# zrlhahaha/Direct12PBRRenderer

Hardware: AMD Instinct MI355X
Metric: shaded Mpixel/s at 4K G-buffer (full deferred frame: clustered shade + bloom + auto-exposure + ACES) (higher is better)
Workload: dtype f32

## Files before the change

### direct12pbrrenderer_amd/csrc/bloom.hip

```cpp
#include <type_traits>
#include "pbr_internal.hpp"
#include "pbr_device.hpp"

using namespace pbr;

__constant__ float c_gauss[9] = {0.0148f, 0.0459f, 0.1050f, 0.1941f, 0.2803f, 0.1941f, 0.1050f, 0.0459f, 0.0148f};

__device__ __forceinline__ float4 to4(F4 v) { return make_float4(v.x, v.y, v.z, v.w); }
__device__ __forceinline__ F4 from4(float4 v) { return f4(v.x, v.y, v.z, v.w); }

struct OutRect { int x0, y0, x1, y1, ox, oy, pitch; };
constexpr int PF_MAX_RECTS = 5;
struct OutRects {
    int n, ox, oy, pitch;
    int x0[PF_MAX_RECTS], y0[PF_MAX_RECTS], x1[PF_MAX_RECTS], y1[PF_MAX_RECTS], tiles_x[PF_MAX_RECTS], first[PF_MAX_RECTS + 1];
};
__global__ __launch_bounds__(256) void k_bloom_prefilter(const pbr_half* __restrict__ hdr, int w, int h, int pitch,
                                                           pbr_half* __restrict__ out, OutRect rc,
                                                           float tx, float ty, float threshold, float knee) {
    const int x = rc.x0 + blockIdx.x * 64 + threadIdx.x;
    const int y = rc.y0 + blockIdx.y * 4 + threadIdx.y;
    if (x >= rc.x1 || y >= rc.y1) return;
    const float u = (float)x * tx, v = (float)y * ty;
    const float ox[5] = {0.0f, -1.0f, -1.0f, 1.0f, 1.0f};
// ... 378 lines not shown
        float fx, hfx, hfy = 0.0f;
        float4 smp[PER_T];
        int ax0, ax1, bx0, bx1;
        tap1d<MODE>(x0 - 4 + lane, iw, ax0, ax1, fx);
        tap1d<MODE>(x0 - 4 + hc, iw, bx0, bx1, hfx);
        const int sx = clampi(x0 - 4 + lane, 0, ow - 1), shx = clampi(x0 - 4 + hc, 0, ow - 1);
        const int first = y0 - 4 + r0;
        const bool shared_rows = MODE == M_UP && first >= 1 && first + PER_T - 1 <= oh - 2;
        if (MODE == M_UP && shared_rows) {
            constexpr int NR = PER_T / 2 + 2;
            const int base = (first >> 1) - 1 + (first & 1);
            V3 hrow[NR];
            const float wx0 = 1.0f - fx;
#pragma unroll
            for (int j = 0; j < NR; j++) {
                const H4* row = reinterpret_cast<const H4*>(in) + (size_t)min(base + j, ih - 1) * iw;
                const H4 c0 = row[ax0], c1 = row[ax1];
                hrow[j] = fma3(h3f(c1), fx, h3f(c0) * wx0);
            }
            auto blend = [&](auto parity) {
                constexpr int P = decltype(parity)::value;
#pragma unroll
                for (int k = 0; k < PER_T; k++) {
                    constexpr int dummy = 0; (void)dummy;
                    const int odd = (P + k) & 1;
                    const int i0 = (P + k + 1) / 2 - P;
                    const float fyk = odd ? 0.25f : 0.75f, wy0 = 1.0f - fyk;
                    const V3 r = fma3(hrow[i0 + 1], fyk, hrow[i0] * wy0);
                    smp[k] = make_float4(r.x, r.y, r.z, 0.0f);
                }
            };
            if (first & 1) blend(std::integral_constant<int, 1>{}); else blend(std::integral_constant<int, 0>{});
#pragma unroll
            for (int k = 0; k < PER_T; k++)
                if (DUAL) up[k] = reinterpret_cast<const H4*>(in2)[(size_t)(first + k) * ow + sx];
        } else {
            Tap2 taps[PER_T];
            float fy[PER_T];
#pragma unroll
            for (int k = 0; k < PER_T; k++) {
                const int jj = clampi(first + k, 0, oh - 1);
                int ay0, ay1;
                tap1d<MODE>(jj, ih, ay0, ay1, fy[k]);
                taps[k] = load_tap2<MODE>(in, iw, ax0, ax1, ay0, ay1);
                if (DUAL) up[k] = reinterpret_cast<const H4*>(in2)[(size_t)jj * ow + sx];
            }
#pragma unroll
            for (int k = 0; k < PER_T; k++) smp[k] = finish_tap2_rgb<MODE>(taps[k], fx, fy[k]);
        }
        if (has_halo) {
            const int jj = clampi(first + hk, 0, oh - 1);
            int ay0, ay1;
            tap1d<MODE>(jj, ih, ay0, ay1, hfy);
            htap = load_tap2<MODE>(in, iw, bx0, bx1, ay0, ay1);
            if (DUAL) hup = reinterpret_cast<const H4*>(in2)[(size_t)jj * ow + shx];
        }
#pragma unroll
        for (int k = 0; k < PER_T; k++) {
            line[lane] = smp[k];
            if (DUAL) line2[lane] = make_float4((float)up[k].x, (float)up[k].y, (float)up[k].z, 0.0f);
            if (has_halo && hk == k) {
                line[hc] = finish_tap2_rgb<MODE>(htap, hfx, hfy);
                if (DUAL) line2[hc] = make_float4((float)hup.x, (float)hup.y, (float)hup.z, 0.0f);
            }
            wave_sync();
            V3 g = gauss9_rgb(line + lane);
            if (DUAL) g = g + gauss9_rgb(line2 + lane);
            wave_sync();
            H4 th;
            th.x = to_half_rn(g.x); th.y = to_half_rn(g.y); th.z = to_half_rn(g.z); th.w = alpha_t;
            sT[r0 + k][lane] = th;
        }
    }
    __syncthreads();
#pragma unroll
    for (int k = 0; k < PER_O; k++) {
        const int r = wv + NW * k, y = y0 + r;
        if (x >= ow || y >= oh) continue;
        V3 a3 = v3(0.0f, 0.0f, 0.0f);
#pragma unroll
        for (int i = 0; i < 9; i++) a3 = fma3(h3f(sT[r + i][lane]), c_gauss[i], a3);
        const F4 a = f4(a3.x, a3.y, a3.z, alpha_v);
        if (TAIL == 0) {
            store_h4(out + 4 * ((size_t)y * out_pitch + x), a);
        } else {
            if (!(in_mx && y >= tr.my0 && y < tr.my1)) continue;
            const half4v a0 = round_h4(a);
            const F4 s = h4f(hdr_in[k]);
            H4 o;
            o.x = to_half_rn(s.x + (float)a0.x); o.y = to_half_rn(s.y + (float)a0.y); o.z = to_half_rn(s.z + (float)a0.z); o.w = to_half_rn(s.w + (float)a0.w);
            *reinterpret_cast<H4*>(out + 4 * ((size_t)(y - tr.by) * out_pitch + (x - tr.bx))) = o;
            if (TAIL == 2) {
                if (x >= tr.hx0 && x < tr.hx1 && y >= tr.hy0 && y < tr.hy1)
                    atomicAdd(&sh_hist[wv][luminance_bin_exact((float)o.x, (float)o.y, (float)o.z, min_log, inv_range)], 1u);
            }
        }
    }
    if (tile + (int)gridDim.x < n_tiles) __syncthreads();
    }
    if (TAIL == 2) {
        __syncthreads();
        for (int i = t; i < PBR_HISTOGRAM_BINS; i += NT) {
            uint32_t sum = 0;
#pragma unroll
            for (int w2 = 0; w2 < NW; w2++) sum += sh_hist[w2][i];
            if (sum) atomicAdd(&hist[i], sum);
        }
    }
}

__device__ __forceinline__ H4 ld_h4(const void* base, uint32_t byte_off) {
    return *reinterpret_cast<const H4*>(reinterpret_cast<const char*>(base) + byte_off);
}
__device__ __forceinline__ void gauss9_pair(const float2* e, float& ge, float& go) {
    const float s[10] = {e[0].x, e[0].y, e[1].x, e[1].y, e[2].x, e[2].y, e[3].x, e[3].y, e[4].x, e[4].y};
    float a = 0.0f, b = 0.0f;
#pragma unroll
    for (int i = 0; i < 9; i++) { a = __builtin_fmaf(s[i], c_gauss[i], a); b = __builtin_fmaf(s[i + 1], c_gauss[i], b); }
    ge = a; go = b;
}

namespace poly {
constexpr double G[9] = {0.0148, 0.0459, 0.1050, 0.1941, 0.2803, 0.1941, 0.1050, 0.0459, 0.0148};
constexpr double g(int k) { return (k < -4 || k > 4) ? 0.0 : G[k + 4]; }
constexpr float E(int j) { return (float)(0.75 * g(2 * j) + 0.25 * g(2 * j + 2) + 0.75 * g(2 * j + 1) + 0.25 * g(2 * j - 1)); }
}

template <bool DUAL, int TAIL, int TH>
__global__ __launch_bounds__(512, 4) void k_blur_up_poly(const pbr_half* __restrict__ in, int iw, int ih,
                                                          const pbr_half* __restrict__ in2,
                                                          pbr_half* __restrict__ out, int ow, int oh, int out_pitch,
                                                          int tiles_x, int n_tiles,
                                                          TailRect tr, float min_log, float inv_range,
                                                          uint32_t* __restrict__ hist) {
    constexpr int TW = 128, NP = TW / 2 + 4, NC = TW / 2 + 6, SR = TH + 8, NT = 512, NW = NT / 64;
    constexpr int NPAIR = TH / 2 + 5;
    constexpr int PPW = (NPAIR + NW - 1) / NW;
    constexpr int PER_O = TH / 4;
    static_assert(TH % 4 == 0 && (PPW + 1) * 6 <= 64 && 2 * PPW * 4 <= 64, "one halo entry per lane");
    __shared__ H4 sLineC[NW][NC + 2];
    __shared__ float2 sLineU[DUAL ? NW : 1][3][NP];
    __shared__ H4 sT[SR][TW];
    __shared__ uint32_t sh_hist[TAIL == 2 ? NW : 1][TAIL == 2 ? PBR_HISTOGRAM_BINS : 1];
    static_assert(sizeof(sLineC) + sizeof(sLineU) + sizeof(sT) + sizeof(sh_hist) <= 80 * 1024, "k_blur_up_poly: two blocks per CU no longer fit the LDS");
    const int t = threadIdx.x, lane = t & 63;
    const int wv = __builtin_amdgcn_readfirstlane(t >> 6);
    const int vc = t & 127, vg = __builtin_amdgcn_readfirstlane(t >> 7);
    if (TAIL == 2) {
        for (int i = t; i < NW * PBR_HISTOGRAM_BINS; i += NT) (&sh_hist[0][0])[i] = 0u;
    }
    const size_t a_at = (size_t)min(tr.my0 >> 1, ih - 1) * iw + min(tr.mx0 >> 1, iw - 1);
    float alpha_h = gauss9_const((float)reinterpret_cast<const H4*>(in)[a_at].w);
    if (DUAL) alpha_h = alpha_h + gauss9_const((float)reinterpret_cast<const H4*>(in2)[(size_t)min(tr.my0, oh - 1) * ow + min(tr.mx0, ow - 1)].w);
    const h16 alpha_t = to_half_rn(alpha_h);
    const float alpha_v = gauss9_const((float)alpha_t);
    const float a0w = (float)to_half_rn(alpha_v);
    auto wave_sync = [] {
        __builtin_amdgcn_fence(__ATOMIC_RELEASE, "wavefront");
        __builtin_amdgcn_wave_barrier();
        __builtin_amdgcn_fence(__ATOMIC_ACQUIRE, "wavefront");
    };
    for (int tile = blockIdx.x; tile < n_tiles; tile += gridDim.x) {
    const int x0 = (tr.tx0 + tile % tiles_x) * TW, y0 = (tr.ty0 + tile / tiles_x) * TH;
    const int xv = x0 + vc, rbase = vg * PER_O;
    H4 hdr_in[PER_O];
    const bool in_mx = TAIL != 0 && xv >= tr.mx0 && xv < tr.mx1;
    char* const hdr_row0 = reinterpret_cast<char*>(out) + (ptrdiff_t)(y0 + rbase - tr.by) * out_pitch * 8;
    const uint32_t hdr_x = (uint32_t)(xv - tr.bx) * 8u;
    const size_t hdr_pitch = (size_t)out_pitch * 8u;
    {
        const int i_first = wv * PPW;
        const int n_pairs = min(PPW, NPAIR - i_first);
        const int cb = (y0 >> 1) - 3 + i_first;
        const uint32_t ccol = (uint32_t)clampi((x0 >> 1) - 3 + lane, 0, iw - 1) * 8u;
        H4 cr[PPW + 1], chalo{};
        const int hk = lane / 6, hq = 64 + lane % 6;
        const bool has_halo = lane < 6 * (PPW + 1);
        H4 upE[DUAL ? 2 * PPW : 1], upO[DUAL ? 2 * PPW : 1], hupE{}, hupO{};
        const int uk = lane >> 2, uq = 64 + (lane & 3);
        const bool has_uhalo = DUAL && lane < 8 * PPW;
        if (n_pairs > 0) {
#pragma unroll
            for (int k = 0; k <= PPW; k++) {
                const char* row = reinterpret_cast<const char*>(in) + (size_t)clampi(cb + k, 0, ih - 1) * iw * 8u;
                cr[k] = ld_h4(row, ccol);
            }
            if (has_halo) {
                const char* row = reinterpret_cast<const char*>(in) + (size_t)clampi(cb + hk, 0, ih - 1) * iw * 8u;
                chalo = ld_h4(row, (uint32_t)clampi((x0 >> 1) - 3 + hq, 0, iw - 1) * 8u);
            }
            if (DUAL) {
                const int sxe = clampi(x0 - 4 + 2 * lane, 0, ow - 1), sxo = clampi(x0 - 3 + 2 * lane, 0, ow - 1);
#pragma unroll
                for (int k = 0; k < 2 * PPW; k++) {
                    const char* row = reinterpret_cast<const char*>(in2) + (size_t)clampi(y0 - 4 + 2 * i_first - 1 + k, 0, oh - 1) * ow * 8u;
                    upE[k] = ld_h4(row, (uint32_t)sxe * 8u); upO[k] = ld_h4(row, (uint32_t)sxo * 8u);
                }
                if (has_uhalo) {
                    const uint32_t row = (uint32_t)(clampi(y0 - 4 + 2 * i_first - 1 + uk, 0, oh - 1) * ow) * 8u;
                    hupE = ld_h4(in2, row + (uint32_t)clampi(x0 - 4 + 2 * uq, 0, ow - 1) * 8u); hupO = ld_h4(in2, row + (uint32_t)clampi(x0 - 3 + 2 * uq, 0, ow - 1) * 8u);
                }
            }
        }
        if (TAIL != 0) {
#pragma unroll
            for (int k = 0; k < PER_O; k++) {
                const int y = y0 + rbase + k;
                if (in_mx && y >= tr.my0 && y < tr.my1) hdr_in[k] = ld_h4(hdr_row0 + k * hdr_pitch, hdr_x);
            }
        }
        if (n_pairs > 0) {
            H4* line = sLineC[wv];
            float2 (*lineU)[NP] = sLineU[DUAL ? wv : 0];
            V3 pE = v3(0.0f, 0.0f, 0.0f), pO = pE;
#pragma unroll
            for (int k = 0; k <= PPW; k++) {
                if (k > n_pairs) break;
                line[lane] = cr[k];
                if (has_halo && hk == k) line[hq] = chalo;
                wave_sync();
                V3 e[7];
#pragma unroll
                for (int j = 0; j < 7; j++) e[j] = h3f(line[lane + j]);
                wave_sync();
                constexpr float PE[6] = {poly::E(-3), poly::E(-2), poly::E(-1), poly::E(0), poly::E(1), poly::E(2)};
                V3 cE = v3(0.0f, 0.0f, 0.0f), cO = cE;
#pragma unroll
                for (int j = 0; j < 6; j++) { cE = fma3(e[j], PE[j], cE); cO = fma3(e[j + 1], PE[5 - j], cO); }
                if (k > 0) {
#pragma unroll
                    for (int half = 0; half < 2; half++) {
                        const int r = 2 * (i_first + k - 1) - 1 + half;
                        if (r < 0 || r >= SR) continue;
                        const float fy = half ? 0.75f : 0.25f, wy0 = 1.0f - fy;
                        V3 bE = fma3(cE, fy, pE * wy0), bO = fma3(cO, fy, pO * wy0);
                        if (DUAL) {
                            const int u = 2 * (k - 1) + half;
                            lineU[0][lane] = make_float2((float)upE[u].x, (float)upO[u].x); lineU[1][lane] = make_float2((float)upE[u].y, (float)upO[u].y);
                            lineU[2][lane] = make_float2((float)upE[u].z, (float)upO[u].z);
                            if (has_uhalo && uk == u) {
                                lineU[0][uq] = make_float2((float)hupE.x, (float)hupO.x); lineU[1][uq] = make_float2((float)hupE.y, (float)hupO.y);
                                lineU[2][uq] = make_float2((float)hupE.z, (float)hupO.z);
                            }
                            wave_sync();
                            V3 uE, uO;
                            gauss9_pair(lineU[0] + lane, uE.x, uO.x); gauss9_pair(lineU[1] + lane, uE.y, uO.y); gauss9_pair(lineU[2] + lane, uE.z, uO.z);
                            wave_sync();
                            bE = bE + uE; bO = bO + uO;
                        }
                        struct alignas(16) H8 { H4 a, b; } th;
                        th.a.x = to_half_rn(bE.x); th.a.y = to_half_rn(bE.y); th.a.z = to_half_rn(bE.z); th.a.w = alpha_t;
                        th.b.x = to_half_rn(bO.x); th.b.y = to_half_rn(bO.y); th.b.z = to_half_rn(bO.z); th.b.w = alpha_t;
                        *reinterpret_cast<H8*>(&sT[r][2 * lane]) = th;
                    }
                }
                pE = cE; pO = cO;
            }
        }
    }
    __syncthreads();
    {
        H4 win[PER_O + 8];
#pragma unroll
        for (int i = 0; i < PER_O + 8; i++) win[i] = sT[rbase + i][vc];
#pragma unroll
        for (int k = 0; k < PER_O; k++) {
            const int y = y0 + rbase + k;
            if (xv >= ow || y >= oh) continue;
            V3 a3 = v3(0.0f, 0.0f, 0.0f);
#pragma unroll
            for (int i = 0; i < 9; i++) a3 = fma3(h3f(win[k + i]), c_gauss[i], a3);
            const F4 a = f4(a3.x, a3.y, a3.z, alpha_v);
            if (TAIL == 0) {
                store_h4(out + 4 * ((size_t)y * out_pitch + xv), a);
            } else {
                if (!(in_mx && y >= tr.my0 && y < tr.my1)) continue;
                const half2v a01 = round_h2(a3.x, a3.y);
                const h16 a2 = to_half_rn(a3.z);
                const F4 s = h4f(hdr_in[k]);
                struct alignas(8) O4 { half2v lo, hi; } o;
                o.lo = round_h2(s.x + (float)a01.x, s.y + (float)a01.y);
                o.hi = round_h2(s.z + (float)a2, s.w + a0w);
                *reinterpret_cast<O4*>(hdr_row0 + k * hdr_pitch + hdr_x) = o;
                if (TAIL == 2) {
                    if (xv >= tr.hx0 && xv < tr.hx1 && y >= tr.hy0 && y < tr.hy1)
                        atomicAdd(&sh_hist[wv][luminance_bin_exact((float)o.lo.x, (float)o.lo.y, (float)o.hi.x, min_log, inv_range)], 1u);
                }
            }
        }
    }
    if (tile + (int)gridDim.x < n_tiles) __syncthreads();
    }
    if (TAIL == 2) {
        __syncthreads();
        for (int i = t; i < PBR_HISTOGRAM_BINS; i += NT) {
            uint32_t sum = 0;
#pragma unroll
            for (int w2 = 0; w2 < NW; w2++) sum += sh_hist[w2][i];
            if (sum) atomicAdd(&hist[i], sum);
        }
    }
}

static int blur_h_rows(uint32_t ow, uint32_t oh) {
    const uint64_t row_blocks = (uint64_t)((ow + 255) / 256) * oh;
    int rows = (int)(row_blocks / 2048);
    return rows < 1 ? 1 : (rows > HB_MAX_ROWS ? HB_MAX_ROWS : rows);
}

static bool exact_half(uint32_t n) { return (n & 1u) == 0u && n <= 8192u; }

template <int MODE, bool DUAL, int TAIL>
static pbr_status launch_hv(pbr_ctx* ctx, const pbr_half* in, uint32_t iw, uint32_t ih, const pbr_half* in2,
                            pbr_half* out, uint32_t ow, uint32_t oh, uint32_t out_pitch,
                            const uint32_t* rect, float min_log, float inv_range, uint32_t* hist,
                            const uint32_t* merge_rect = nullptr, const uint32_t* buf_origin = nullptr) {
    TailRect tr;
    tr.hx0 = rect ? (int)rect[0] : 0; tr.hy0 = rect ? (int)rect[1] : 0;
    tr.hx1 = rect ? (int)(rect[0] + rect[2]) : 0; tr.hy1 = rect ? (int)(rect[1] + rect[3]) : 0;
    tr.mx0 = merge_rect ? (int)merge_rect[0] : 0; tr.my0 = merge_rect ? (int)merge_rect[1] : 0;
    tr.mx1 = merge_rect ? (int)(merge_rect[0] + merge_rect[2]) : (int)ow; tr.my1 = merge_rect ? (int)(merge_rect[1] + merge_rect[3]) : (int)oh;
    tr.bx = buf_origin ? (int)buf_origin[0] : 0; tr.by = buf_origin ? (int)buf_origin[1] : 0;
    static const int hist_blocks = pbr::knob_int("PBR_BLOOM_HIST_BLOCKS", 1024);
    auto even_blocks = [](int n_tiles) { const int per = (n_tiles + hist_blocks - 1) / hist_blocks; return (n_tiles + per - 1) / per; };
    if constexpr (MODE == M_UP) {
        static const int wide_forced = pbr::knob_int("PBR_BLOOM_WIDE", -1);
        const int wtx0 = tr.mx0 / 128, wty0 = tr.my0 / 32;
        const int wtiles_x = (tr.mx1 + 127) / 128 - wtx0, wn = wtiles_x * ((tr.my1 + 31) / 32 - wty0);
        if (wide_forced >= 0 ? wide_forced == 1 : (wn >= 400 && !ctx->bloom_shader_order)) {
            tr.tx0 = wtx0; tr.ty0 = wty0;
            hipLaunchKernelGGL((k_blur_up_poly<DUAL, TAIL, 32>), dim3(TAIL == 2 ? even_blocks(wn) : wn), dim3(512), 0, ctx->stream,
                               in, (int)iw, (int)ih, in2, out, (int)ow, (int)oh, (int)out_pitch, wtiles_x, wn, tr, min_log, inv_range, hist);
            return launched(ctx, "k_blur_up_poly");
        }
    }
    const bool big = (uint64_t)((tr.mx1 + 63) / 64 - tr.mx0 / 64) * ((tr.my1 + 31) / 32 - tr.my0 / 32) >= 900;
    const int th = big ? 32 : 16;
    tr.tx0 = tr.mx0 / 64; tr.ty0 = tr.my0 / th;
    const int tiles_x = (tr.mx1 + 63) / 64 - tr.tx0;
    const int n_tiles = tiles_x * ((tr.my1 + th - 1) / th - tr.ty0);
    const int blocks = TAIL == 2 ? even_blocks(n_tiles) : n_tiles;
    if (big) {
        hipLaunchKernelGGL((k_blur_hv<MODE, DUAL, TAIL, 32, 512>), dim3(blocks), dim3(512), 0, ctx->stream,
                           in, (int)iw, (int)ih, in2, out, (int)ow, (int)oh, (int)out_pitch, tiles_x, n_tiles, tr, min_log, inv_range, hist);
    } else {
        hipLaunchKernelGGL((k_blur_hv<MODE, DUAL, TAIL, 16, 512>), dim3(blocks), dim3(512), 0, ctx->stream,
                           in, (int)iw, (int)ih, in2, out, (int)ow, (int)oh, (int)out_pitch, tiles_x, n_tiles, tr, min_log, inv_range, hist);
    }
    return launched(ctx, "k_blur_hv");
}

extern "C" {

static pbr_status prefilter_launch(pbr_ctx* ctx, const pbr_half* hdr, uint32_t w, uint32_t h, uint32_t pitch,
                                   pbr_half* out, const OutRect* rcs, int n, float threshold, float knee) {
    const uint32_t ow = w >> 1, oh = h >> 1;
    const float tx = 1.0f / (float)ow, ty = 1.0f / (float)oh;
    if (exact_half(w) && exact_half(h)) {
        OutRects rs{};
        rs.n = n; rs.ox = rcs[0].ox; rs.oy = rcs[0].oy; rs.pitch = rcs[0].pitch;
        int blocks = 0;
        for (int r = 0; r < n; r++) {
            rs.x0[r] = rcs[r].x0; rs.y0[r] = rcs[r].y0; rs.x1[r] = rcs[r].x1; rs.y1[r] = rcs[r].y1;
            rs.tiles_x[r] = (rcs[r].x1 - rcs[r].x0 + PF_TW - 1) / PF_TW;
            rs.first[r] = blocks;
            blocks += rs.tiles_x[r] * ((rcs[r].y1 - rcs[r].y0 + PF_TH - 1) / PF_TH);
        }
        rs.first[n] = blocks;
        hipLaunchKernelGGL(k_bloom_prefilter_2x, dim3(blocks), dim3(256), 0, ctx->stream, hdr, (int)w, (int)h, (int)pitch, out, rs, threshold, knee);
        return launched(ctx, "k_bloom_prefilter_2x");
    }
    for (int r = 0; r < n; r++) {
        const uint32_t rw = (uint32_t)(rcs[r].x1 - rcs[r].x0), rh = (uint32_t)(rcs[r].y1 - rcs[r].y0);
        dim3 grid((rw + 63) / 64, (rh + 3) / 4);
        hipLaunchKernelGGL(k_bloom_prefilter, grid, dim3(64, 4), 0, ctx->stream, hdr, (int)w, (int)h, (int)pitch, out, rcs[r], tx, ty, threshold, knee);
        pbr_status st = launched(ctx, "k_bloom_prefilter");
        if (st) return st;
    }
    return PBR_OK;
}

pbr_status pbr_bloom_prefilter(pbr_ctx* ctx, const pbr_half* hdr, uint32_t w, uint32_t h, uint32_t pitch,
                               pbr_half* out, float threshold, float knee) {
    if (!ctx) return PBR_ERR_INVALID;
    PBR_REQUIRE(ctx, hdr && out, "pbr_bloom_prefilter: null pointer");
    PBR_REQUIRE(ctx, (w >> 1) >= 1 && (h >> 1) >= 1 && w <= 65535 && h <= 65535 && pitch >= w, "pbr_bloom_prefilter: bad size");
    const OutRect rc{0, 0, (int)(w >> 1), (int)(h >> 1), 0, 0, (int)(w >> 1)};
    return prefilter_launch(ctx, hdr, w, h, pitch, out, &rc, 1, threshold, knee);
}

pbr_status pbr_bloom_prefilter_rect(pbr_ctx* ctx, const pbr_half* hdr, uint32_t w, uint32_t h, uint32_t pitch,
                                    pbr_half* out, uint32_t out_pitch, uint32_t out_x, uint32_t out_y,
                                    const uint32_t rect[4], float threshold, float knee) {
    if (!ctx) return PBR_ERR_INVALID;
    PBR_REQUIRE(ctx, hdr && out && rect, "pbr_bloom_prefilter_rect: null pointer");
    PBR_REQUIRE(ctx, (w >> 1) >= 1 && (h >> 1) >= 1 && w <= 65535 && h <= 65535 && pitch >= w, "pbr_bloom_prefilter_rect: bad size");
    PBR_REQUIRE(ctx, rect[2] >= 1 && rect[3] >= 1 && rect[0] + rect[2] <= (w >> 1) && rect[1] + rect[3] <= (h >> 1), "pbr_bloom_prefilter_rect: rect outside the half-res image");
    PBR_REQUIRE(ctx, out_pitch >= out_x + rect[0] + rect[2] && out_pitch <= 65535 && out_y <= 65535, "pbr_bloom_prefilter_rect: rect does not fit the output pitch");
    const OutRect rc{(int)rect[0], (int)rect[1], (int)(rect[0] + rect[2]), (int)(rect[1] + rect[3]), (int)out_x, (int)out_y, (int)out_pitch};
    return prefilter_launch(ctx, hdr, w, h, pitch, out, &rc, 1, threshold, knee);
}

pbr_status pbr_bloom_prefilter_rects(pbr_ctx* ctx, const pbr_half* hdr, uint32_t w, uint32_t h, uint32_t pitch,
                                     pbr_half* out, uint32_t out_pitch, uint32_t out_x, uint32_t out_y,
                                     const uint32_t (*rects)[4], uint32_t n_rects, float threshold, float knee) {
    if (!ctx) return PBR_ERR_INVALID;
    PBR_REQUIRE(ctx, hdr && out && rects && n_rects >= 1 && n_rects <= (uint32_t)PF_MAX_RECTS, "pbr_bloom_prefilter_rects: null pointer / 1 .. 5 rectangles");
    PBR_REQUIRE(ctx, (w >> 1) >= 1 && (h >> 1) >= 1 && w <= 65535 && h <= 65535 && pitch >= w && out_pitch <= 65535 && out_y <= 65535, "pbr_bloom_prefilter_rects: bad size");
    OutRect rcs[PF_MAX_RECTS];
    for (uint32_t r = 0; r < n_rects; r++) {
        const uint32_t* q = rects[r];
        PBR_REQUIRE(ctx, q[2] >= 1 && q[3] >= 1 && q[0] + q[2] <= (w >> 1) && q[1] + q[3] <= (h >> 1) && out_pitch >= out_x + q[0] + q[2],
                    "pbr_bloom_prefilter_rects: rectangle outside the half-res image / the output pitch");
        rcs[r] = OutRect{(int)q[0], (int)q[1], (int)(q[0] + q[2]), (int)(q[1] + q[3]), (int)out_x, (int)out_y, (int)out_pitch};
    }
    return prefilter_launch(ctx, hdr, w, h, pitch, out, rcs, (int)n_rects, threshold, knee);
}

pbr_status pbr_blur_h(pbr_ctx* ctx, const pbr_half* in, uint32_t iw, uint32_t ih, pbr_half* out, uint32_t ow, uint32_t oh) {
    if (!ctx) return PBR_ERR_INVALID;
    PBR_REQUIRE(ctx, in && out, "pbr_blur_h: null pointer");
    PBR_REQUIRE(ctx, iw && ih && ow && oh && iw <= 65535 && ih <= 65535 && ow <= 65535 && oh <= 65535, "pbr_blur_h: bad size");
    const float tx = 1.0f / (float)ow, ty = 1.0f / (float)oh;
    const int rows = blur_h_rows(ow, oh);
    dim3 grid((ow + 255) / 256, (oh + rows - 1) / rows);
    hipLaunchKernelGGL(k_blur_h<false>, grid, dim3(256), 0, ctx->stream, in, (int)iw, (int)ih, (const pbr_half*)nullptr, 0, 0, out, (int)ow, (int)oh, tx, ty, rows);
    return launched(ctx, "k_blur_h");
}

pbr_status pbr_blur_v(pbr_ctx* ctx, const pbr_half* in, uint32_t iw, uint32_t ih, pbr_half* out, uint32_t ow, uint32_t oh) {
    if (!ctx) return PBR_ERR_INVALID;
    PBR_REQUIRE(ctx, in && out, "pbr_blur_v: null pointer");
    PBR_REQUIRE(ctx, iw && ih && ow && oh && iw <= 65535 && ih <= 65535 && ow <= 65535 && oh <= 65535, "pbr_blur_v: bad size");
    const float tx = 1.0f / (float)ow, ty = 1.0f / (float)oh;
    dim3 grid((ow + VT_W - 1) / VT_W, (oh + VT_R - 1) / VT_R);
    hipLaunchKernelGGL(k_blur_v, grid, dim3(VT_W, 4), 0, ctx->stream, in, (int)iw, (int)ih, out, (int)ow, (int)oh, tx, ty);
    return launched(ctx, "k_blur_v");
}

pbr_status pbr_bloom_upsample_add(pbr_ctx* ctx, const pbr_half* upper, uint32_t uw, uint32_t uh,
                                  const pbr_half* lower, uint32_t lw, uint32_t lh, pbr_half* out) {
    if (!ctx) return PBR_ERR_INVALID;
    PBR_REQUIRE(ctx, upper && lower && out, "pbr_bloom_upsample_add: null pointer");
    PBR_REQUIRE(ctx, uw && uh && lw && lh && uw <= 65535 && uh <= 65535, "pbr_bloom_upsample_add: bad size");
    const float tx = 1.0f / (float)uw, ty = 1.0f / (float)uh;
    const int rows = blur_h_rows(uw, uh);
    dim3 grid((uw + 255) / 256, (uh + rows - 1) / rows);
    hipLaunchKernelGGL(k_blur_h<true>, grid, dim3(256), 0, ctx->stream, lower, (int)lw, (int)lh, upper, (int)uw, (int)uh, out, (int)uw, (int)uh, tx, ty, rows);
    return launched(ctx, "k_blur_h<dual>");
}

pbr_status pbr_bloom_merge(pbr_ctx* ctx, pbr_half* hdr, uint32_t pitch, const pbr_half* in, uint32_t w, uint32_t h) {
    if (!ctx) return PBR_ERR_INVALID;
    PBR_REQUIRE(ctx, hdr && in, "pbr_bloom_merge: null pointer");
    PBR_REQUIRE(ctx, w && h && w <= 65535 && h <= 65535 && pitch >= w, "pbr_bloom_merge: bad size");
    dim3 grid((w + 255) / 256, h);
    hipLaunchKernelGGL(k_bloom_merge, grid, dim3(256), 0, ctx->stream, hdr, (int)pitch, in, (int)w, (int)h);
    return launched(ctx, "k_bloom_merge");
}

pbr_status pbr_bloom_up_level(pbr_ctx* ctx, const pbr_half* upper, const pbr_half* lower, uint32_t lw, uint32_t lh,
                              pbr_half* out, uint32_t ow, uint32_t oh) {
    if (!ctx) return PBR_ERR_INVALID;
    PBR_REQUIRE(ctx, lower && out && out != lower && out != upper, "pbr_bloom_up_level: null pointer / out aliases an input");
    PBR_REQUIRE(ctx, lw >= 1 && lh >= 1 && ow == 2 * lw && oh == 2 * lh && exact_half(ow) && exact_half(oh), "pbr_bloom_up_level: out must be exactly twice lower, even, <= 8192");
    if (upper) return launch_hv<M_UP, true, 0>(ctx, lower, lw, lh, upper, out, ow, oh, ow, nullptr, 0.0f, 0.0f, nullptr);
    return launch_hv<M_UP, false, 0>(ctx, lower, lw, lh, nullptr, out, ow, oh, ow, nullptr, 0.0f, 0.0f, nullptr);
}

static pbr_status bloom_final(pbr_ctx* ctx, const pbr_half* b0, pbr_half* hdr, uint32_t w, uint32_t h, uint32_t pitch,
                              const uint32_t* hist_rect, float min_log, float inv_range, uint32_t* hist256) {
    const float tx = 1.0f / (float)w, ty = 1.0f / (float)h;
    const int tiles_x = (int)((w + VT_W - 1) / VT_W), tiles_y = (int)((h + VT_R - 1) / VT_R);
    int blocks = tiles_x * tiles_y;
    if (blocks > 1280) blocks = 1280;
    if (hist256) {
        hipLaunchKernelGGL(k_blur_v_merge<true>, dim3(blocks), dim3(VT_W, 4), 0, ctx->stream, b0, (int)w, (int)h, tx, ty, hdr, (int)pitch, tiles_x, tiles_y,
                           (int)hist_rect[0], (int)hist_rect[1], (int)(hist_rect[0] + hist_rect[2]), (int)(hist_rect[1] + hist_rect[3]), min_log, inv_range, hist256);
    } else {
        hipLaunchKernelGGL(k_blur_v_merge<false>, dim3(blocks), dim3(VT_W, 4), 0, ctx->stream, b0, (int)w, (int)h, tx, ty, hdr, (int)pitch, tiles_x, tiles_y,
                           0, 0, 0, 0, 0.0f, 0.0f, (uint32_t*)nullptr);
    }
    return launched(ctx, "k_blur_v_merge");
}

static pbr_status bloom_pyramid(pbr_ctx* ctx, uint32_t w, uint32_t h, pbr_half* A, pbr_half* B, const pbr_half** res_out, const uint32_t* need0 = nullptr) {
    auto a = [&](uint32_t l) { return A + 4 * pbr_bloom_level_offset(w, h, l); };
    auto b = [&](uint32_t l) { return B + 4 * pbr_bloom_level_offset(w, h, l); };
    auto W = [&](uint32_t l) { return w >> l; };
    auto H = [&](uint32_t l) { return h >> l; };
    pbr_status r;
    auto exact = [&](uint32_t l) { return exact_half(W(l)) && exact_half(H(l)); };
    for (uint32_t i = 0; i < PBR_BLOOM_STEP; i++) {
        const uint32_t up = i + 1, lo = i + 2;
        if (exact(up)) {
            if ((r = launch_hv<M_DOWN, false, 0>(ctx, a(up), W(up), H(up), nullptr, a(lo), W(lo), H(lo), W(lo), nullptr, 0.0f, 0.0f, nullptr))) return r;
        } else {
            if ((r = pbr_blur_h(ctx, a(up), W(up), H(up), b(lo), W(lo), H(lo)))) return r;
            if ((r = pbr_blur_v(ctx, b(lo), W(lo), H(lo), a(lo), W(lo), H(lo)))) return r;
        }
    }
    uint32_t need[PBR_BLOOM_MIPS][4];
    static const bool shrink = pbr::knob_int("PBR_BLOOM_SHRINK", 1) != 0;
    const bool use_need = need0 != nullptr && shrink;
    if (use_need) {
        int x0 = (int)need0[0], y0 = (int)need0[1], x1 = (int)(need0[0] + need0[2]), y1 = (int)(need0[1] + need0[3]);
        for (uint32_t l = 1; l < PBR_BLOOM_MIPS; l++) {
            x0 = (x0 - 4) / 2 - 2; y0 = (y0 - 4) / 2 - 2; x1 = (x1 + 4 + 1) / 2 + 2; y1 = (y1 + 4 + 1) / 2 + 2;
            const int cx0 = x0 < 0 ? 0 : x0, cy0 = y0 < 0 ? 0 : y0, cx1 = x1 > (int)W(l) ? (int)W(l) : x1, cy1 = y1 > (int)H(l) ? (int)H(l) : y1;
            need[l][0] = (uint32_t)cx0; need[l][1] = (uint32_t)cy0; need[l][2] = (uint32_t)(cx1 - cx0); need[l][3] = (uint32_t)(cy1 - cy0);
            x0 = cx0; y0 = cy0; x1 = cx1; y1 = cy1;
        }
    }
    const pbr_half* res = a(PBR_BLOOM_MIPS - 1);
    for (int i = PBR_BLOOM_STEP - 1; i >= 0; i--) {
        const uint32_t up = (uint32_t)i + 1;
        if (exact(up)) {
            if ((r = launch_hv<M_UP, true, 0>(ctx, res, W(up + 1), H(up + 1), a(up), b(up), W(up), H(up), W(up), nullptr, 0.0f, 0.0f, nullptr,
                                              use_need ? need[up] : nullptr))) return r;
            res = b(up);
        } else {
            if ((r = pbr_bloom_upsample_add(ctx, a(up), W(up), H(up), res, W(up + 1), H(up + 1), b(up)))) return r;
            if ((r = pbr_blur_v(ctx, b(up), W(up), H(up), a(up), W(up), H(up)))) return r;
            res = a(up);
        }
    }
    *res_out = res;
    return PBR_OK;
}

static pbr_status bloom_impl(pbr_ctx* ctx, pbr_half* hdr, uint32_t w, uint32_t h, uint32_t pitch, pbr_half* A, pbr_half* B,
                             float threshold, float knee, const uint32_t* hist_rect, float min_log, float inv_range, uint32_t* hist256) {
    PBR_REQUIRE(ctx, hdr && A && B, "pbr_bloom: null pointer");
    PBR_REQUIRE(ctx, (w >> (PBR_BLOOM_MIPS - 1)) >= 1 && (h >> (PBR_BLOOM_MIPS - 1)) >= 1, "pbr_bloom: image too small for 5 mips");
    PBR_REQUIRE(ctx, w <= 65535 && h <= 65535 && pitch >= w, "pbr_bloom: bad size");
    pbr_status r;
    if ((r = pbr_bloom_prefilter(ctx, hdr, w, h, pitch, A + 4 * pbr_bloom_level_offset(w, h, 1), threshold, knee))) return r;
    const pbr_half* res = nullptr;
    if ((r = bloom_pyramid(ctx, w, h, A, B, &res))) return r;
    if (exact_half(w) && exact_half(h)) {
        if (hist256) return launch_hv<M_UP, false, 2>(ctx, res, w >> 1, h >> 1, nullptr, hdr, w, h, pitch, hist_rect, min_log, inv_range, hist256);
        return launch_hv<M_UP, false, 1>(ctx, res, w >> 1, h >> 1, nullptr, hdr, w, h, pitch, nullptr, 0.0f, 0.0f, nullptr);
    }
    pbr_half* b0 = B;
    if ((r = pbr_blur_h(ctx, res, w >> 1, h >> 1, b0, w, h))) return r;
    return bloom_final(ctx, b0, hdr, w, h, pitch, hist_rect, min_log, inv_range, hist256);
}

pbr_status pbr_bloom(pbr_ctx* ctx, pbr_half* hdr, uint32_t w, uint32_t h, uint32_t pitch,
                     pbr_half* A, pbr_half* B, float threshold, float knee) {
    if (!ctx) return PBR_ERR_INVALID;
    return bloom_impl(ctx, hdr, w, h, pitch, A, B, threshold, knee, nullptr, 0.0f, 0.0f, nullptr);
}

pbr_status pbr_bloom_histogram(pbr_ctx* ctx, pbr_half* hdr, uint32_t w, uint32_t h, uint32_t pitch,
                               pbr_half* A, pbr_half* B, float threshold, float knee,
                               const uint32_t rect[4], float min_log, float inv_range, uint32_t* hist256) {
    if (!ctx) return PBR_ERR_INVALID;
    PBR_REQUIRE(ctx, rect && hist256, "pbr_bloom_histogram: null pointer");
    PBR_REQUIRE(ctx, rect[2] >= 1 && rect[3] >= 1 && rect[0] + rect[2] <= w && rect[1] + rect[3] <= h, "pbr_bloom_histogram: rect outside the image");
    return bloom_impl(ctx, hdr, w, h, pitch, A, B, threshold, knee, rect, min_log, inv_range, hist256);
}

pbr_status pbr_bloom_tiled(pbr_ctx* ctx, pbr_half* hdr, uint32_t hdr_pitch, const uint32_t hdr_rect[4],
                           uint32_t ew, uint32_t eh, pbr_half* A, pbr_half* B, const uint32_t merge_rect[4],
                           float min_log, float inv_range, uint32_t* hist256) {
    if (!ctx) return PBR_ERR_INVALID;
    PBR_REQUIRE(ctx, hdr && hdr_rect && A && B && merge_rect, "pbr_bloom_tiled: null pointer");
    PBR_REQUIRE(ctx, ew <= 65535 && eh <= 65535 && (ew >> (PBR_BLOOM_MIPS - 1)) >= 1 && (eh >> (PBR_BLOOM_MIPS - 1)) >= 1, "pbr_bloom_tiled: bad size");
    PBR_REQUIRE(ctx, hdr_rect[2] >= 1 && hdr_rect[3] >= 1 && hdr_rect[0] + hdr_rect[2] <= ew && hdr_rect[1] + hdr_rect[3] <= eh && hdr_pitch >= hdr_rect[2],
                "pbr_bloom_tiled: hdr_rect outside the extended tile");
    PBR_REQUIRE(ctx, merge_rect[2] >= 1 && merge_rect[3] >= 1 && merge_rect[0] >= hdr_rect[0] && merge_rect[1] >= hdr_rect[1] &&
                     merge_rect[0] + merge_rect[2] <= hdr_rect[0] + hdr_rect[2] && merge_rect[1] + merge_rect[3] <= hdr_rect[1] + hdr_rect[3],
                "pbr_bloom_tiled: merge_rect outside hdr_rect");
    if (!exact_half(ew) || !exact_half(eh))
        return pbr::fail(ctx, PBR_ERR_UNSUPPORTED, "pbr_bloom_tiled: the extended tile must be even and <= 8192 on a side");
    const pbr_half* res = nullptr;
    pbr_status r;
    if ((r = bloom_pyramid(ctx, ew, eh, A, B, &res, merge_rect))) return r;
    const uint32_t origin[2] = {hdr_rect[0], hdr_rect[1]};
    if (hist256) return launch_hv<M_UP, false, 2>(ctx, res, ew >> 1, eh >> 1, nullptr, hdr, ew, eh, hdr_pitch, merge_rect, min_log, inv_range, hist256, merge_rect, origin);
    return launch_hv<M_UP, false, 1>(ctx, res, ew >> 1, eh >> 1, nullptr, hdr, ew, eh, hdr_pitch, nullptr, 0.0f, 0.0f, nullptr, merge_rect, origin);
}

}
```

Measured before the change: 17640.

## Fuse last bloom upsample level into final upsample-merge-histogram tail kernel

Adds a kernel that computes the level-1 bloom upsample (level-2 upsample plus level-1 blur) in shared memory and feeds it straight into the final full-resolution upsample, HDR merge and luminance histogram. The level-1 intermediate is no longer written to and reread from global memory, and one launch disappears. The fused path is used when a histogram is requested, the sizes halve exactly and the poly path would be chosen. The cost is recomputing halo regions per tile and heavy LDS use, which may limit occupancy.

Result: no change. 17660, median of 5 (+0.1%).

```diff
diff --git a/direct12pbrrenderer_amd/csrc/bloom.hip b/direct12pbrrenderer_amd/csrc/bloom.hip
--- a/direct12pbrrenderer_amd/csrc/bloom.hip
+++ b/direct12pbrrenderer_amd/csrc/bloom.hip
@@ -704,6 +704,188 @@
     }
 }
 
+namespace up1 {
+constexpr int TW = 128, TH = 32, NT = 512, NW = NT / 64;
+constexpr int R1 = TH / 2 + 6, C1 = TW / 2 + 6, C1P = C1 + 2;
+constexpr int RH = R1 + 8, CH = TW / 2 + 8, NQ = CH / 2;
+constexpr int R2 = RH / 2 + 1, C2 = NQ + 6;
+constexpr int RD = RH, CD = CH + 8;
+constexpr int NS2 = R2 * C2, NSTAGE = NS2 + RD * CD;
+constexpr int NPAIR_H = RH / 2;
+constexpr int SR = TH + 8, NPAIR = TH / 2 + 5, PPW = (NPAIR + NW - 1) / NW, PER_O = TH / 4;
+static_assert(NSTAGE % NT == 0, "staging loads split evenly over the block");
+static_assert(RH % 2 == 0 && NPAIR + 1 <= R1, "region sizes");
+}
+
+__global__ __launch_bounds__(512, 4) void k_bloom_up1_tail(const pbr_half* __restrict__ l2, int w2, int h2,
+                                                            const pbr_half* __restrict__ l1d, int w1, int h1,
+                                                            pbr_half* __restrict__ out, int ow, int oh, int out_pitch,
+                                                            int tiles_x, int n_tiles,
+                                                            TailRect tr, float min_log, float inv_range,
+                                                            uint32_t* __restrict__ hist) {
+    using namespace up1;
+    struct Front { H4 stage[NSTAGE]; H4 hd[RH][CH]; };
+    union Big { Front f; H4 sT[SR][TW]; };
+    __shared__ Big big;
+    __shared__ H4 sL1[R1][C1P];
+    __shared__ uint32_t sh_hist[NW][PBR_HISTOGRAM_BINS];
+    static_assert(sizeof(Big) + sizeof(sL1) + sizeof(sh_hist) <= 80 * 1024, "k_bloom_up1_tail: two blocks per CU no longer fit the LDS");
+    H4 (*const stage2)[C2] = reinterpret_cast<H4 (*)[C2]>(big.f.stage);
+    H4 (*const staged)[CD] = reinterpret_cast<H4 (*)[CD]>(big.f.stage + NS2);
+    const int t = threadIdx.x, lane = t & 63;
+    const int wv = __builtin_amdgcn_readfirstlane(t >> 6);
+    const int vc = t & 127, vg = __builtin_amdgcn_readfirstlane(t >> 7);
+    for (int i = t; i < NW * PBR_HISTOGRAM_BINS; i += NT) (&sh_hist[0][0])[i] = 0u;
+    const float alpha_hd = gauss9_const((float)reinterpret_cast<const H4*>(l2)[0].w) + gauss9_const((float)reinterpret_cast<const H4*>(l1d)[0].w);
+    const h16 alpha_td = to_half_rn(alpha_hd);
+    const h16 alpha_l1 = to_half_rn(gauss9_const((float)alpha_td));
+    const h16 alpha_t = to_half_rn(gauss9_const((float)alpha_l1));
+    const float alpha_v = gauss9_const((float)alpha_t);
+    const float a0w = (float)to_half_rn(alpha_v);
+    constexpr float PE[6] = {poly::E(-3), poly::E(-2), poly::E(-1), poly::E(0), poly::E(1), poly::E(2)};
+    for (int tile = blockIdx.x; tile < n_tiles; tile += gridDim.x) {
+    const int x0 = (tile % tiles_x) * TW, y0 = (tile / tiles_x) * TH;
+    const int xv = x0 + vc, rbase = vg * PER_O;
+    {
+        H4 v[NSTAGE / NT];
+#pragma unroll
+        for (int k = 0; k < NSTAGE / NT; k++) {
+            const int j = t + NT * k;
+            const pbr_half* base;
+            uint32_t off;
+            if (j < NS2) {
+                const int r = j / C2, c = j - r * C2;
+                base = l2; off = ((uint32_t)clampi((y0 >> 2) - 4 + r, 0, h2 - 1) * (uint32_t)w2 + (uint32_t)clampi((x0 >> 2) - 5 + c, 0, w2 - 1)) * 8u;
+            } else {
+                const int r = (j - NS2) / CD, c = (j - NS2) - r * CD;
+                base = l1d; off = ((uint32_t)clampi((y0 >> 1) - 7 + r, 0, h1 - 1) * (uint32_t)w1 + (uint32_t)clampi((x0 >> 1) - 8 + c, 0, w1 - 1)) * 8u;
+            }
+            v[k] = ld_h4(base, off);
+        }
+#pragma unroll
+        for (int k = 0; k < NSTAGE / NT; k++) big.f.stage[t + NT * k] = v[k];
+    }
+    H4 hdr_in[PER_O];
+    const bool in_mx = xv >= tr.mx0 && xv < tr.mx1;
+    char* const hdr_row0 = reinterpret_cast<char*>(out) + (ptrdiff_t)(y0 + rbase - tr.by) * out_pitch * 8;
+    const uint32_t hdr_x = (uint32_t)(xv - tr.bx) * 8u;
+    const size_t hdr_pitch = (size_t)out_pitch * 8u;
+#pragma unroll
+    for (int k = 0; k < PER_O; k++) {
+        const int y = y0 + rbase + k;
+        if (in_mx && y >= tr.my0 && y < tr.my1) hdr_in[k] = ld_h4(hdr_row0 + k * hdr_pitch, hdr_x);
+    }
+    __syncthreads();
+    for (int it = t; it < NPAIR_H * NQ; it += NT) {
+        const int i = it / NQ, q = it - i * NQ;
+        V3 fE[2], fO[2];
+#pragma unroll
+        for (int m = 0; m < 2; m++) {
+            V3 e[7];
+#pragma unroll
+            for (int j = 0; j < 7; j++) e[j] = h3f(stage2[i + m][q + j]);
+            V3 cE = v3(0.0f, 0.0f, 0.0f), cO = cE;
+#pragma unroll
+            for (int j = 0; j < 6; j++) { cE = fma3(e[j], PE[j], cE); cO = fma3(e[j + 1], PE[5 - j], cO); }
+            fE[m] = cE; fO[m] = cO;
+        }
+#pragma unroll
+        for (int half = 0; half < 2; half++) {
+            const int r = 2 * i + half;
+            const float fy = half ? 0.75f : 0.25f, wy0 = 1.0f - fy;
+            V3 bE = fma3(fE[1], fy, fE[0] * wy0), bO = fma3(fO[1], fy, fO[0] * wy0);
+            V3 s[10];
+#pragma unroll
+            for (int j = 0; j < 10; j++) s[j] = h3f(staged[r][2 * q + j]);
+            V3 uE = v3(0.0f, 0.0f, 0.0f), uO = uE;
+#pragma unroll
+            for (int j = 0; j < 9; j++) { uE = fma3(s[j], c_gauss[j], uE); uO = fma3(s[j + 1], c_gauss[j], uO); }
+            bE = bE + uE; bO = bO + uO;
+            struct alignas(16) H8 { H4 a, b; } th;
+            th.a.x = to_half_rn(bE.x); th.a.y = to_half_rn(bE.y); th.a.z = to_half_rn(bE.z); th.a.w = alpha_td;
+            th.b.x = to_half_rn(bO.x); th.b.y = to_half_rn(bO.y); th.b.z = to_half_rn(bO.z); th.b.w = alpha_td;
+            *reinterpret_cast<H8*>(&big.f.hd[r][2 * q]) = th;
+        }
+    }
+    __syncthreads();
+    for (int it = t; it < R1 * C1; it += NT) {
+        const int i = it / C1, e = it - i * C1;
+        const int hr = clampi((y0 >> 1) - 3 + i, 0, h1 - 1) - (y0 >> 1) + 3;
+        const int hc = clampi((x0 >> 1) - 3 + e, 0, w1 - 1) - (x0 >> 1) + 4;
+        V3 a3 = v3(0.0f, 0.0f, 0.0f);
+#pragma unroll
+        for (int j = 0; j < 9; j++) a3 = fma3(h3f(big.f.hd[hr + j][hc]), c_gauss[j], a3);
+        H4 o;
+        o.x = to_half_rn(a3.x); o.y = to_half_rn(a3.y); o.z = to_half_rn(a3.z); o.w = alpha_l1;
+        sL1[i][e] = o;
+    }
+    __syncthreads();
+    {
+        const int i_first = wv * PPW;
+        const int n_pairs = min(PPW, NPAIR - i_first);
+        if (n_pairs > 0) {
+            V3 pE = v3(0.0f, 0.0f, 0.0f), pO = pE;
+#pragma unroll
+            for (int k = 0; k <= PPW; k++) {
+                if (k > n_pairs) break;
+                V3 e[7];
+#pragma unroll
+                for (int j = 0; j < 7; j++) e[j] = h3f(sL1[i_first + k][lane + j]);
+                V3 cE = v3(0.0f, 0.0f, 0.0f), cO = cE;
+#pragma unroll
+                for (int j = 0; j < 6; j++) { cE = fma3(e[j], PE[j], cE); cO = fma3(e[j + 1], PE[5 - j], cO); }
+                if (k > 0) {
+#pragma unroll
+                    for (int half = 0; half < 2; half++) {
+                        const int r = 2 * (i_first + k - 1) - 1 + half;
+                        if (r < 0 || r >= SR) continue;
+                        const float fy = half ? 0.75f : 0.25f, wy0 = 1.0f - fy;
+                        const V3 bE = fma3(cE, fy, pE * wy0), bO = fma3(cO, fy, pO * wy0);
+                        struct alignas(16) H8 { H4 a, b; } th;
+                        th.a.x = to_half_rn(bE.x); th.a.y = to_half_rn(bE.y); th.a.z = to_half_rn(bE.z); th.a.w = alpha_t;
+                        th.b.x = to_half_rn(bO.x); th.b.y = to_half_rn(bO.y); th.b.z = to_half_rn(bO.z); th.b.w = alpha_t;
+                        *reinterpret_cast<H8*>(&big.sT[r][2 * lane]) = th;
+                    }
+                }
+                pE = cE; pO = cO;
+            }
+        }
+    }
+    __syncthreads();
+    {
+        H4 win[PER_O + 8];
+#pragma unroll
+        for (int i = 0; i < PER_O + 8; i++) win[i] = big.sT[rbase + i][vc];
+#pragma unroll
+        for (int k = 0; k < PER_O; k++) {
+            const int y = y0 + rbase + k;
+            if (xv >= ow || y >= oh) continue;
+            if (!(in_mx && y >= tr.my0 && y < tr.my1)) continue;
+            V3 a3 = v3(0.0f, 0.0f, 0.0f);
+#pragma unroll
+            for (int i = 0; i < 9; i++) a3 = fma3(h3f(win[k + i]), c_gauss[i], a3);
+            const half2v a01 = round_h2(a3.x, a3.y);
+            const h16 a2 = to_half_rn(a3.z);
+            const F4 s = h4f(hdr_in[k]);
+            struct alignas(8) O4 { half2v lo, hi; } o;
+            o.lo = round_h2(s.x + (float)a01.x, s.y + (float)a01.y);
+            o.hi = round_h2(s.z + (float)a2, s.w + a0w);
+            *reinterpret_cast<O4*>(hdr_row0 + k * hdr_pitch + hdr_x) = o;
+            if (xv >= tr.hx0 && xv < tr.hx1 && y >= tr.hy0 && y < tr.hy1)
+                atomicAdd(&sh_hist[wv][luminance_bin_exact((float)o.lo.x, (float)o.lo.y, (float)o.hi.x, min_log, inv_range)], 1u);
+        }
+    }
+    if (tile + (int)gridDim.x < n_tiles) __syncthreads();
+    }
+    __syncthreads();
+    for (int i = t; i < PBR_HISTOGRAM_BINS; i += NT) {
+        uint32_t sum = 0;
+#pragma unroll
+        for (int wi = 0; wi < NW; wi++) sum += sh_hist[wi][i];
+        if (sum) atomicAdd(&hist[i], sum);
+    }
+}
+
 static int blur_h_rows(uint32_t ow, uint32_t oh) {
     const uint64_t row_blocks = (uint64_t)((ow + 255) / 256) * oh;
     int rows = (int)(row_blocks / 2048);
@@ -711,6 +893,17 @@
 }
 
 static bool exact_half(uint32_t n) { return (n & 1u) == 0u && n <= 8192u; }
+
+static int even_blocks(int n_tiles) {
+    static const int hist_blocks = pbr::knob_int("PBR_BLOOM_HIST_BLOCKS", 1024);
+    const int per = (n_tiles + hist_blocks - 1) / hist_blocks;
+    return (n_tiles + per - 1) / per;
+}
+static bool up_poly(const pbr_ctx* ctx, int n_tiles) {
+    static const int wide_forced = pbr::knob_int("PBR_BLOOM_WIDE", -1);
+    return wide_forced >= 0 ? wide_forced == 1 : (n_tiles >= 400 && !ctx->bloom_shader_order);
+}
+static int poly_tiles(uint32_t w, uint32_t h) { return (int)(((w + 127) / 128) * ((h + 31) / 32)); }
 
 template <int MODE, bool DUAL, int TAIL>
 static pbr_status launch_hv(pbr_ctx* ctx, const pbr_half* in, uint32_t iw, uint32_t ih, const pbr_half* in2,
@@ -723,13 +916,10 @@
     tr.mx0 = merge_rect ? (int)merge_rect[0] : 0; tr.my0 = merge_rect ? (int)merge_rect[1] : 0;
     tr.mx1 = merge_rect ? (int)(merge_rect[0] + merge_rect[2]) : (int)ow; tr.my1 = merge_rect ? (int)(merge_rect[1] + merge_rect[3]) : (int)oh;
     tr.bx = buf_origin ? (int)buf_origin[0] : 0; tr.by = buf_origin ? (int)buf_origin[1] : 0;
-    static const int hist_blocks = pbr::knob_int("PBR_BLOOM_HIST_BLOCKS", 1024);
-    auto even_blocks = [](int n_tiles) { const int per = (n_tiles + hist_blocks - 1) / hist_blocks; return (n_tiles + per - 1) / per; };
     if constexpr (MODE == M_UP) {
-        static const int wide_forced = pbr::knob_int("PBR_BLOOM_WIDE", -1);
         const int wtx0 = tr.mx0 / 128, wty0 = tr.my0 / 32;
         const int wtiles_x = (tr.mx1 + 127) / 128 - wtx0, wn = wtiles_x * ((tr.my1 + 31) / 32 - wty0);
-        if (wide_forced >= 0 ? wide_forced == 1 : (wn >= 400 && !ctx->bloom_shader_order)) {
+        if (up_poly(ctx, wn)) {
             tr.tx0 = wtx0; tr.ty0 = wty0;
             hipLaunchKernelGGL((k_blur_up_poly<DUAL, TAIL, 32>), dim3(TAIL == 2 ? even_blocks(wn) : wn), dim3(512), 0, ctx->stream,
                                in, (int)iw, (int)ih, in2, out, (int)ow, (int)oh, (int)out_pitch, wtiles_x, wn, tr, min_log, inv_range, hist);
@@ -886,7 +1076,8 @@
     return launched(ctx, "k_blur_v_merge");
 }
 
-static pbr_status bloom_pyramid(pbr_ctx* ctx, uint32_t w, uint32_t h, pbr_half* A, pbr_half* B, const pbr_half** res_out, const uint32_t* need0 = nullptr) {
+static pbr_status bloom_pyramid(pbr_ctx* ctx, uint32_t w, uint32_t h, pbr_half* A, pbr_half* B, const pbr_half** res_out, const uint32_t* need0 = nullptr,
+                                uint32_t last_up = 1) {
     auto a = [&](uint32_t l) { return A + 4 * pbr_bloom_level_offset(w, h, l); };
     auto b = [&](uint32_t l) { return B + 4 * pbr_bloom_level_offset(w, h, l); };
     auto W = [&](uint32_t l) { return w >> l; };
@@ -915,7 +1106,7 @@
         }
     }
     const pbr_half* res = a(PBR_BLOOM_MIPS - 1);
-    for (int i = PBR_BLOOM_STEP - 1; i >= 0; i--) {
+    for (int i = PBR_BLOOM_STEP - 1; i >= (int)last_up - 1; i--) {
         const uint32_t up = (uint32_t)i + 1;
         if (exact(up)) {
             if ((r = launch_hv<M_UP, true, 0>(ctx, res, W(up + 1), H(up + 1), a(up), b(up), W(up), H(up), W(up), nullptr, 0.0f, 0.0f, nullptr,
@@ -939,6 +1130,19 @@
     pbr_status r;
     if ((r = pbr_bloom_prefilter(ctx, hdr, w, h, pitch, A + 4 * pbr_bloom_level_offset(w, h, 1), threshold, knee))) return r;
     const pbr_half* res = nullptr;
+    const uint32_t w1 = w >> 1, h1 = h >> 1;
+    if (hist256 && exact_half(w) && exact_half(h) && exact_half(w1) && exact_half(h1) && up_poly(ctx, poly_tiles(w1, h1)) && up_poly(ctx, poly_tiles(w, h))) {
+        if ((r = bloom_pyramid(ctx, w, h, A, B, &res, nullptr, 2))) return r;
+        TailRect tr{};
+        tr.mx1 = (int)w; tr.my1 = (int)h;
+        tr.hx0 = (int)hist_rect[0]; tr.hy0 = (int)hist_rect[1];
+        tr.hx1 = (int)(hist_rect[0] + hist_rect[2]); tr.hy1 = (int)(hist_rect[1] + hist_rect[3]);
+        const int tiles_x = (int)((w + up1::TW - 1) / up1::TW), n_tiles = tiles_x * (int)((h + up1::TH - 1) / up1::TH);
+        hipLaunchKernelGGL(k_bloom_up1_tail, dim3(even_blocks(n_tiles)), dim3(up1::NT), 0, ctx->stream,
+                           res, (int)(w1 >> 1), (int)(h1 >> 1), A + 4 * pbr_bloom_level_offset(w, h, 1), (int)w1, (int)h1,
+                           hdr, (int)w, (int)h, (int)pitch, tiles_x, n_tiles, tr, min_log, inv_range, hist256);
+        return launched(ctx, "k_bloom_up1_tail");
+    }
     if ((r = bloom_pyramid(ctx, w, h, A, B, &res))) return r;
     if (exact_half(w) && exact_half(h)) {
         if (hist256) return launch_hv<M_UP, false, 2>(ctx, res, w >> 1, h >> 1, nullptr, hdr, w, h, pitch, hist_rect, min_log, inv_range, hist256);
```
